# arunsethuraman/multiclust

Measured on AMD Instinct MI355X. Metric: EM iterations/sec, IxLxK admixture, higher is better.
Workload: dtype f64; 1 GPU; c3: 10000 diploid x 100000 loci, M_l~U{2,3,4}, admixture K=8, SQUAREM-3 (-s 3); I=10000, L=100000, T=300302, ploidy=2, K=8, accel_scheme=3, units=1 initialisation(s), one per GPU

## Files before the change

multiclust_amd/csrc/mchip.hip:

```cpp
#include "mchip_context.h"
#include "mchip_finalize.h"

#include <math.h>
#include <stdio.h>
#include <stdlib.h>
#include <string.h>
#include <sys/syscall.h>
#include <unistd.h>

mchip_progress_slot mchip_progress_slots[MCHIP_PROGRESS_SLOTS];
std::atomic<unsigned long long> mchip_progress_events{0};
static std::atomic<int> progress_next_slot{0};

mchip_progress_slot *mchip_progress_my_slot(void)
{
	static thread_local mchip_progress_slot *mine = nullptr;
	if (!mine) {
		int x = progress_next_slot.fetch_add(1, std::memory_order_relaxed);
		if (x >= MCHIP_PROGRESS_SLOTS) x = MCHIP_PROGRESS_SLOTS - 1;
		mine = &mchip_progress_slots[x];
		mine->tid.store((long)syscall(SYS_gettid), std::memory_order_relaxed);
	}
	return mine;
}
// ... 18 lines not shown
		mchip_ktable_get_17, mchip_ktable_get_18, mchip_ktable_get_19, mchip_ktable_get_20, mchip_ktable_get_21, mchip_ktable_get_22, mchip_ktable_get_23, mchip_ktable_get_24,
		mchip_ktable_get_25, mchip_ktable_get_26, mchip_ktable_get_27, mchip_ktable_get_28, mchip_ktable_get_29, mchip_ktable_get_30, mchip_ktable_get_31, mchip_ktable_get_32,
		mchip_ktable_get_33, mchip_ktable_get_34, mchip_ktable_get_35, mchip_ktable_get_36, mchip_ktable_get_37, mchip_ktable_get_38, mchip_ktable_get_39, mchip_ktable_get_40,
		mchip_ktable_get_41, mchip_ktable_get_42, mchip_ktable_get_43, mchip_ktable_get_44, mchip_ktable_get_45, mchip_ktable_get_46, mchip_ktable_get_47, mchip_ktable_get_48,
		mchip_ktable_get_49, mchip_ktable_get_50, mchip_ktable_get_51, mchip_ktable_get_52, mchip_ktable_get_53, mchip_ktable_get_54, mchip_ktable_get_55, mchip_ktable_get_56,
		mchip_ktable_get_57, mchip_ktable_get_58, mchip_ktable_get_59, mchip_ktable_get_60, mchip_ktable_get_61, mchip_ktable_get_62, mchip_ktable_get_63, mchip_ktable_get_64,
	};
	static_assert(MCHIP_MAX_K == 64, "one kernel translation unit per K (Makefile: KS)");
	return (K >= 1 && K <= MCHIP_MAX_K) ? tabs[K]() : nullptr;
}

static void read_knobs(mchip_context *ctx)
{
	auto on = [](const char *name) { return getenv(name) != nullptr ? 1 : 0; };
	auto num = [](const char *name, int dflt) { const char *e = getenv(name); return (e && atoi(e) > 0) ? atoi(e) : dflt; };
	ctx->knob.no_bial = on("MCHIP_NO_BIAL");
	ctx->knob.no_counts = on("MCHIP_NO_COUNTS");
	ctx->knob.force_dense = on("MCHIP_FORCE_DENSE");
	ctx->knob.force_safe = on("MCHIP_FORCE_SAFE");
	ctx->knob.no_graph = on("MCHIP_NO_GRAPH");
	ctx->knob.no_dual = on("MCHIP_NO_DUAL");
	ctx->knob.no_slab_sum = on("MCHIP_NO_SLAB_SUM");
	ctx->knob.no_fused_finalize = on("MCHIP_NO_FUSED_FINALIZE");
	ctx->knob.no_col_split = on("MCHIP_NO_COL_SPLIT");
	ctx->knob.part_no_tile = on("MCHIP_PART_NO_TILE");
	ctx->knob.sim_no_tile = on("MCHIP_SIM_NO_TILE");
	const int both = num("MCHIP_BLOCKS_PER_CU", 64);
	ctx->knob.per_cu_col = num("MCHIP_BLOCKS_PER_CU_COL", both);
	ctx->knob.per_cu_ind = num("MCHIP_BLOCKS_PER_CU_IND", both);
	const char *f = getenv("MCHIP_SLAB_FRAC");
	ctx->knob.slab_frac = (f && atof(f) > 0) ? atof(f) : 0.3;
	ctx->knob.no_roundup = on("MCHIP_NO_CHUNK_ROUNDUP");
	ctx->knob.geometry_given = on("MCHIP_BLOCKS_PER_CU") || on("MCHIP_BLOCKS_PER_CU_COL") || on("MCHIP_SLAB_FRAC");
}


constexpr int RT_I = 64;

__global__ __launch_bounds__(256) void k_relayout(const uint8_t *__restrict__ raw, int I, int L, int pl, const int32_t *__restrict__ ua,
			   int limit, uint8_t *gtA, uint8_t *gtS, int n_ltiles, int RT_L, int *bad)
{
	extern __shared__ __attribute__((aligned(16))) uint8_t tile[];
	const int rowb = RT_L * pl;
	const int l0 = (blockIdx.x % n_ltiles) * RT_L, i0 = (blockIdx.x / n_ltiles) * RT_I;
	int flags = 0;
	const int roww = rowb / 4;
// ... 747 lines not shown
	else { idx -= nq; pdst[idx] = cyc[1] ? p_if_accepted[idx] : p_otherwise[idx]; }
}

int check_slot(mchip_context *ctx, int slot)
{
	if (!ctx) return MCHIP_ERR_INVALID;
	if (!ctx->K) return fail(ctx, MCHIP_ERR_STATE, "no model set%s", nullptr);
	if (slot < 0 || slot > 2) return fail(ctx, MCHIP_ERR_INVALID, "slot out of range%s", nullptr);
	return MCHIP_OK;
}

static void prof_mark(mchip_context *ctx, int kind, bool start)
{
	if (!ctx->profiling) return;
	if (ctx->ev_used >= ctx->ev_pool.size()) {
		hipEvent_t e;
		if (hipEventCreate(&e) != hipSuccess) return;
		ctx->ev_pool.push_back(e);
	}
	(void)hipEventRecord(ctx->ev_pool[ctx->ev_used++], ctx->stream);
	if (start) ctx->ev_kind.push_back(kind);
}

static void drop_graphs(mchip_context *ctx)
{
	for (int s = 0; s < 3; s++)
		if (ctx->step_graph[s]) { (void)MCHIP_WAIT(hipGraphExecDestroy(ctx->step_graph[s])); ctx->step_graph[s] = nullptr; }
	for (int s = 0; s < 3; s++)
		for (int m = 0; m < 5; m++)
			if (ctx->cycle_graph[s][m]) { (void)MCHIP_WAIT(hipGraphExecDestroy(ctx->cycle_graph[s][m])); ctx->cycle_graph[s][m] = nullptr; }
}

void free_model(mchip_context *ctx)
{
	drop_graphs(ctx);
	for (int s = 0; s < 3; s++) { dfree(ctx->d_p[s]); dfree(ctx->d_q[s]); }
	for (int s = 0; s < MCHIP_MAX_SECANTS; s++) { dfree(ctx->d_up[s]); dfree(ctx->d_vp[s]); dfree(ctx->d_uq[s]); dfree(ctx->d_vq[s]); }
	dfree(ctx->d_sik); dfree(ctx->d_stage); dfree(ctx->d_logp); dfree(ctx->d_Apart); dfree(ctx->d_Spart); dfree(ctx->d_llpart); dfree(ctx->d_llpart2);
	dfree(ctx->d_redpart); dfree(ctx->d_flags);
	ctx->K = 0;
	ctx->parked_K = 0;
	ctx->kt = nullptr;
	ctx->have_ll = 0;
	ctx->s_cache_slot = -1;
}

// ... 98 lines not shown
	    MCHIP_WAIT(hipMalloc((void **)&ctx->d_run, sizeof(mchip_run_state))) != hipSuccess ||
	    MCHIP_WAIT(hipMalloc((void **)&ctx->d_cyc, 4 * sizeof(int))) != hipSuccess ||
	    MCHIP_WAIT(hipEventCreate(&ctx->ev_begin)) != hipSuccess || MCHIP_WAIT(hipEventCreate(&ctx->ev_end)) != hipSuccess) {
		delete ctx;
		return MCHIP_ERR_ALLOC;
	}
	*out = ctx;
	return MCHIP_OK;
}

int mchip_destroy(mchip_context *ctx)
{
	MCHIP_ENTRY();
	if (!ctx) return MCHIP_OK;
	(void)MCHIP_WAIT(hipSetDevice(ctx->device));
	(void)MCHIP_WAIT(hipStreamSynchronize(ctx->stream));
	free_model(ctx);
	free_data(ctx);
	dfree(ctx->d_scalars);
	dfree(ctx->d_cyc);
	dfree(ctx->d_run);
	if (ctx->h_pinned) (void)MCHIP_WAIT(hipHostFree(ctx->h_pinned));
	for (hipEvent_t e : ctx->ev_pool) (void)MCHIP_WAIT(hipEventDestroy(e));
	(void)MCHIP_WAIT(hipEventDestroy(ctx->ev_begin));
	(void)MCHIP_WAIT(hipEventDestroy(ctx->ev_end));
	(void)MCHIP_WAIT(hipStreamDestroy(ctx->stream));
	delete ctx;
	return MCHIP_OK;
}

const char *mchip_last_error(const mchip_context *ctx) { return ctx ? ctx->err : "null context"; }

int mchip_synchronize(mchip_context *ctx)
{
	MCHIP_ENTRY();
	if (!ctx) return MCHIP_ERR_INVALID;
	HIPCHK(hipStreamSynchronize(ctx->stream));
	return MCHIP_OK;
}

int mchip_device_info(mchip_context *ctx, char *name, int name_len, int *compute_units, double *hbm_bytes)
{
	MCHIP_ENTRY();
	if (!ctx) return MCHIP_ERR_INVALID;
	hipDeviceProp_t prop;
	HIPCHK(hipGetDeviceProperties(&prop, ctx->device));
// ... 597 lines not shown
		int rc = finalize_shared_eta(ctx, to, stop);
		if (rc) return rc;
		mchip_pass_args b = pass_args(ctx, from);
		b.Q = ctx->d_sik;
		b.qstride = ctx->K;
		b.stop = stop;
		prof_mark(ctx, MCHIP_KERN_ACCUM_P, true);
		ctx->kt->mix_column(b, ctx->stream);
		prof_mark(ctx, MCHIP_KERN_ACCUM_P, false);
		launch_finalize_p(ctx, ctx->kt->col_slabs(b, 1), ctx->d_Apart, from, to, 0, ctx->p_lb, ctx->do_projection, stop);
	}
	HIPCHK(hipGetLastError());
	if (mode == 0) ctx->have_ll = 1;
	return MCHIP_OK;
}

static int run_estep(mchip_context *ctx, int from, int to, int do_mstep, const int *stop = nullptr, const int *skip_ind = nullptr,
		     bool defer_ll = false)
{
	if (!ctx->admixture) return run_mixture(ctx, from, to, do_mstep, 0, stop, -1, defer_ll);
	mchip_pass_args a = pass_args(ctx, from);
	a.stop = stop;
	a.skip_ind = skip_ind;
	if (do_mstep || !ctx->sparse) {
		prof_mark(ctx, MCHIP_KERN_ACCUM_P, true);
		if (do_mstep) ctx->kt->accum_p(a, ctx->stream); else ctx->kt->loglik(a, ctx->stream);
		prof_mark(ctx, MCHIP_KERN_ACCUM_P, false);
	}
	if (ctx->sparse && do_mstep && !stop && ctx->s_cache_slot == from) {
		HIPCHK(hipMemcpyAsync(ctx->d_scalars, ctx->d_scalars + 2, sizeof(double), hipMemcpyDeviceToDevice, ctx->stream));
	} else {
		prof_mark(ctx, MCHIP_KERN_ACCUM_Q, true);
		ctx->kt->accum_q(a, ctx->stream);
		prof_mark(ctx, MCHIP_KERN_ACCUM_Q, false);
		ctx->ll_parts = ctx->kt->ind_ll_parts(a);
		if (!defer_ll)
			hipLaunchKernelGGL(k_reduce_sum, dim3(1), dim3(MCHIP_BLOCK), 0, ctx->stream, ctx->d_llpart, ctx->ll_parts, ctx->d_scalars, stop);
	}
	ctx->s_cache_slot = -1;
	const int indiv = ctx->qstride != 0;
	const int s_slabs = ctx->kt->ind_slabs(a), n_slabs = ctx->kt->col_slabs(a, 0);
	const int p_loci = finalize_p_loci(ctx->K, ctx->max_M);
	if (do_mstep && indiv && p_loci && !(n_slabs > 8 && !ctx->knob.no_slab_sum) && !ctx->knob.no_fused_finalize) {
		mchip_finalize_p_args p;
		p.L = ctx->L; p.K = ctx->K; p.T = ctx->T; p.loci_per_block = p_loci; p.n_slabs = n_slabs; p.weighted = 1;
		p.do_projection = ctx->do_projection; p.toff = ctx->d_toff; p.Apart = ctx->d_Apart; p.Pfrom = ctx->d_p[from];
		p.Pto = ctx->d_p[to]; p.add_lb = 0.0; p.lb = ctx->p_lb;
		ctx->kt->finalize_qp(ctx->I, s_slabs, ctx->d_Spart, ctx->d_q[from], ctx->qstride, ctx->d_q[to], ctx->d_sik,
				     ctx->do_projection, ctx->eta_lb, p, stop, ctx->stream);
		ctx->empty_rows_nan[to] = 1;
		HIPCHK(hipGetLastError());
		ctx->have_ll = 1;
// ... 587 lines not shown
	if (n_terms < 0 || (n_terms && (!v_index || !coef_a || !coef_b))) return MCHIP_ERR_INVALID;
	for (int t = 0; t < n_terms; t++) if ((rc = check_secant(ctx, v_index[t]))) return rc;
	HIPCHK(hipSetDevice(ctx->device));
	const size_t KT = (size_t)ctx->K * ctx->T;
	hipLaunchKernelGGL(k_add, dim3(nblk(KT)), dim3(256), 0, ctx->stream, ctx->d_p[base], ctx->d_up[u_index], ctx->d_p[to], KT);
	hipLaunchKernelGGL(k_add, dim3(nblk(ctx->nq)), dim3(256), 0, ctx->stream, ctx->d_q[base], ctx->d_uq[u_index], ctx->d_q[to], (size_t)ctx->nq);
	for (int t = 0; t < n_terms; t++) {
		hipLaunchKernelGGL(k_axpy2, dim3(nblk(KT)), dim3(256), 0, ctx->stream, ctx->d_vp[v_index[t]], ctx->d_p[to], KT, coef_a[t], coef_b[t]);
		hipLaunchKernelGGL(k_axpy2, dim3(nblk(ctx->nq)), dim3(256), 0, ctx->stream, ctx->d_vq[v_index[t]], ctx->d_q[to], (size_t)ctx->nq, coef_a[t], coef_b[t]);
	}
	HIPCHK(hipGetLastError());
	ctx->empty_rows_nan[to] = ctx->empty_rows_nan[base];
	return project_slot(ctx, to);
}

int mchip_profile_begin(mchip_context *ctx)
{
	MCHIP_ENTRY();
	if (!ctx) return MCHIP_ERR_INVALID;
	HIPCHK(hipSetDevice(ctx->device));
	ctx->profiling = 1;
	ctx->ev_used = 0;
	ctx->ev_kind.clear();
	HIPCHK(hipEventRecord(ctx->ev_begin, ctx->stream));
	return MCHIP_OK;
}

int mchip_profile_end(mchip_context *ctx, double *total_ms, double *kernel_ms, int *launches)
{
	MCHIP_ENTRY();
	if (!ctx) return MCHIP_ERR_INVALID;
	if (!ctx->profiling) return fail(ctx, MCHIP_ERR_STATE, "profile_end without profile_begin%s", nullptr);
	HIPCHK(hipSetDevice(ctx->device));
	HIPCHK(hipEventRecord(ctx->ev_end, ctx->stream));
	HIPCHK(hipEventSynchronize(ctx->ev_end));
	ctx->profiling = 0;
	float ms = 0;
	HIPCHK(hipEventElapsedTime(&ms, ctx->ev_begin, ctx->ev_end));
	if (total_ms) *total_ms = ms;
	double km[MCHIP_KERN_COUNT] = {0}, longest[MCHIP_KERN_COUNT] = {0};
	int kl[MCHIP_KERN_COUNT] = {0};
	std::vector<float> each(ctx->ev_kind.size(), 0.0f);
	for (size_t p = 0; 2 * p + 1 < ctx->ev_used && p < ctx->ev_kind.size(); p++) {
		HIPCHK(hipEventElapsedTime(&each[p], ctx->ev_pool[2 * p], ctx->ev_pool[2 * p + 1]));
		if (each[p] > longest[ctx->ev_kind[p]]) longest[ctx->ev_kind[p]] = each[p];
	}
	for (size_t p = 0; 2 * p + 1 < ctx->ev_used && p < ctx->ev_kind.size(); p++) {
		const int kind = ctx->ev_kind[p];
		if (each[p] < 0.05 * longest[kind]) continue;
		km[kind] += each[p];
		kl[kind]++;
	}
	for (int x = 0; x < MCHIP_KERN_COUNT; x++) {
		if (kernel_ms) kernel_ms[x] = km[x];
		if (launches) launches[x] = kl[x];
	}
	return MCHIP_OK;
}

int mchip_progress_note(const char *what)
{
	mchip_progress_slot *s = mchip_progress_my_slot();
	s->note.store(what, std::memory_order_relaxed);
	s->since_ns.store(mchip_progress_now(), std::memory_order_relaxed);
	mchip_progress_events.fetch_add(1, std::memory_order_relaxed);
	return MCHIP_OK;
}

int mchip_progress_report(char *buf, int buf_len, unsigned long long *events)
{
	if (events) *events = mchip_progress_events.load(std::memory_order_relaxed);
	if (!buf || buf_len <= 0) return MCHIP_OK;
// ... 20 lines not shown
```

multiclust_amd/csrc/mchip_context.h:

```cpp
#ifndef MCHIP_CONTEXT_H
#define MCHIP_CONTEXT_H

#include "mchip_internal.h"
#include "mchip_progress.h"

#include <functional>
#include <type_traits>
#include <stdio.h>
#include <string.h>

constexpr int RNG_LAG = 31;
constexpr int RNG_CHUNK = 4 * RNG_LAG * 32;

struct saved_set {
	uint8_t *d_raw = nullptr;
	int L = 0;
	std::vector<int32_t> ua;
	std::vector<int> empty;
};

struct mchip_context {
	int device;
	hipStream_t stream;
	char err[512];
// ... 29 lines not shown
	unsigned long long *d_cand_off;
	size_t cand_span_bytes, cand_loci, cand_center_bytes;
	uint32_t *d_jump_hi, *d_jump_lo;
	size_t n_jump_hi;
	struct lattice { uint32_t *d_i, *d_r; uint64_t A, B; unsigned nA, nB; } lat[2];
	uint32_t *d_part_slabs;
	size_t part_slab_bytes;
	uint8_t *d_sim_cluster;
	uint32_t *d_cen_part, *d_cen_work;
	size_t cen_part_bytes, cen_work_bytes;
	int K, admixture, constrained, do_projection, nsec, nq, qstride;
	double eta_lb, p_lb;
	const mchip_ktable *kt;
	double *d_p[3], *d_q[3];
	double *d_up[MCHIP_MAX_SECANTS], *d_vp[MCHIP_MAX_SECANTS], *d_uq[MCHIP_MAX_SECANTS], *d_vq[MCHIP_MAX_SECANTS];
	double *d_sik;
	double *d_stage;
	double *d_logp;
	int ichunk, n_ichunks, lchunk, n_lchunks, n_llpart, flush_blocks, safe_rcp, sparse;
	int ind_waves;
	int xcd_rows;
	struct {
		int no_bial, no_counts, force_dense, force_safe, no_graph, no_dual, no_slab_sum, no_col_split, part_no_tile, sim_no_tile;
		int no_fused_finalize;
		int per_cu_col, per_cu_ind, geometry_given, no_roundup;
		double slab_frac;
	} knob;
	double *d_Apart, *d_Spart, *d_llpart, *d_scalars;
	double *d_llpart2;
	double *d_redpart;
	uint8_t *d_flags;
	double *h_pinned;
	mchip_run_state *d_run;
	hipGraphExec_t step_graph[3];
	hipGraphExec_t cycle_graph[3][5];
	int *d_cyc;
	int have_ll;
	int ll_parts;
	int s_cache_slot;
	int profiling;
	hipEvent_t ev_begin, ev_end;
	std::vector<hipEvent_t> ev_pool;
	std::vector<int> ev_kind;
	size_t ev_used;
};

static int fail(mchip_context *ctx, int code, const char *fmt, const char *detail)
{
	if (ctx) snprintf(ctx->err, sizeof ctx->err, fmt, detail ? detail : "");
	return code;
}

#define HIPCHK(call)                                                                                  \
	do {                                                                                          \
		hipError_t e_ = MCHIP_WAIT(call);                                                     \
		if (e_ != hipSuccess) {                                                               \
			snprintf(ctx->err, sizeof ctx->err, "%s failed: %s (%s:%d)", #call,           \
				 hipGetErrorString(e_), __FILE__, __LINE__);                          \
			return MCHIP_ERR_HIP;                                                         \
		}                                                                                     \
	} while (0)

template <typename Tp> static void dfree(Tp *&p)
{
	if (p) (void)MCHIP_WAIT(hipFree(p));
	p = nullptr;
}
// ... 74 lines not shown
```

multiclust_amd/csrc/mchip_internal.h:

```cpp
#ifndef MCHIP_INTERNAL_H
#define MCHIP_INTERNAL_H

#include <hip/hip_runtime.h>
#include <stdint.h>
#include <vector>
#include "multiclust_hip.h"

#define MCHIP_BLOCK 256
#define MCHIP_SPARSE_MAX_M 32
#ifndef MCHIP_QBLOCK
#define MCHIP_QBLOCK 128
#endif

#ifdef MCHIP_FORCE_SPLIT1
constexpr int mchip_ind_split(int) { return 1; }
#else
constexpr int mchip_ind_split(int K) { return K <= 27 ? 1 : (K <= 48 ? 2 : 4); }
#endif
#ifdef MCHIP_FORCE_SPLIT1
constexpr int mchip_qblock(int) { return MCHIP_QBLOCK; }
#else
constexpr int mchip_qblock(int K) { return K > 48 ? 2 * MCHIP_QBLOCK : MCHIP_QBLOCK; }
#endif
#ifndef MCHIP_COL_SPLIT2_ABOVE
// ... 47 lines not shown
	const double *Q;
	int qstride;
	int ichunk, n_ichunks;
	double *Apart;
	double *llpart;
	int flush_blocks;
	int safe_rcp;
	int lchunk, n_lchunks;
	double *Spart;
	int xcd_rows;
	int no_col_split;
	int ind_waves;
	int sparse;
	int tile_cols;
	int biallelic;
	const int *stop;
	const int *skip_ind;
	const double *P2, *Q2;
	double *llpart2;
	const uint8_t *asA, *asS;
	int part_counts;
};

struct mchip_finalize_p_args {
	int L, K, T, loci_per_block, n_slabs, weighted, do_projection;
	const int32_t *toff;
	const double *Apart, *Pfrom;
	double *Pto;
	double add_lb, lb;
};

struct mchip_ktable {
	void (*accum_p)(const mchip_pass_args &a, hipStream_t s);
	void (*loglik)(const mchip_pass_args &a, hipStream_t s);
	void (*accum_q)(const mchip_pass_args &a, hipStream_t s);
	void (*part_p)(const mchip_pass_args &a, hipStream_t s);
	void (*part_q)(const mchip_pass_args &a, hipStream_t s);
	void (*finalize_q)(int I, int K, int n_lchunks, const double *Spart, const double *Qfrom, int qstride_from,
			   double *Qto, double *sik, int do_mstep, int weighted, int do_projection, double lb, const int *stop, hipStream_t s,
			   double add);
	void (*project_q)(int nrows, int K, double *Q, double lb, const int *stop, hipStream_t s);
	void (*mix_gather)(const mchip_pass_args &a, hipStream_t s);
	void (*mix_finalize)(int I, int n_lchunks, const double *Vpart, const double *eta, double *vik, double *llpart, int mode,
			     const int *stop, hipStream_t s);
	void (*mix_column)(const mchip_pass_args &a, hipStream_t s);
	int (*dual_available)(const mchip_pass_args &a);
	void (*accum_q_dual)(const mchip_pass_args &a, hipStream_t s);
	int (*col_slabs)(const mchip_pass_args &a, int mix);
	int (*ind_slabs)(const mchip_pass_args &a);
	int (*ind_ll_parts)(const mchip_pass_args &a);
	void (*finalize_qp)(int I, int n_slabs_q, const double *Spart, const double *Qfrom, int qstride_from, double *Qto, double *sik,
			    int do_projection_q, double lb_q, const mchip_finalize_p_args &p, const int *stop, hipStream_t s);
};

const mchip_ktable *mchip_get_ktable(int K);

inline int mchip_ind_waves(int K, int tile_cols)
{
	const size_t per_wave = (size_t)(K <= 12 ? 4 : 2) * ((((size_t)tile_cols * (size_t)mchip_kp(K) + 127) / 128) * 128) * sizeof(double);
	for (int w = MCHIP_IND_WAVES_MAX; w > 1; w >>= 1)
		if ((size_t)w * per_wave <= 48 * 1024) return w;
	return 1;
}
__host__ __device__ inline int mchip_ind_slabs(const mchip_pass_args &a) { return (a.n_lchunks + a.ind_waves - 1) / a.ind_waves; }
__host__ __device__ inline int mchip_col_slabs(const mchip_pass_args &a) { return (a.n_ichunks + MCHIP_COL_WAVES - 1) / MCHIP_COL_WAVES; }

#endif
```

multiclust_amd/csrc/mchip_kernels_k.hip:

```cpp
#include "mchip_internal.h"
#include "mchip_finalize.h"

#ifndef MCHIP_K
#error "compile with -DMCHIP_K=<K>"
#endif

namespace {

constexpr int K = MCHIP_K;

__device__ __forceinline__ double rcp_full(double t)
{
	const double r = __builtin_amdgcn_rcp(t);
	const double e = __builtin_fma(-t, r, 1.0);
	const double p = __builtin_fma(e, e, e);
	return __builtin_fma(r, p, r);
}

__device__ __forceinline__ void rcp4(const double (&t)[4], double (&rc)[4])
{
	const double p01 = t[0] * t[1], p23 = t[2] * t[3];
	const double rp = rcp_full(p01 * p23);
	const double r01 = rp * p23, r23 = rp * p01;
	rc[0] = r01 * t[1];
// ... 168 lines not shown
		if (LL && !SAFE) {
			if (++blk >= a.flush_blocks) {
				blk = 0;
				if (prod < 1e-100) {
					ll += log(prod);
					prod = 1.0;
				}
			}
		}
		g = gn;
	}
	if (ACCUM && valid) {
		double *out = a.Apart + ((size_t)blockIdx.y * a.T + c) * K;
#pragma unroll
		for (int k = 0; k < K; k++) out[k] = acc[k];
	}
	if (LL) {
		ll += log(prod);
		const double tot = block_sum<MCHIP_BLOCK>(ll, red);
		if (threadIdx.x == 0) a.llpart[(size_t)blockIdx.y * gridDim.x + blockIdx.x] = tot;
	}
}

template <int BITS, bool MIX, bool SAFE = false>
__global__ __launch_bounds__(MCHIP_BLOCK) void k_column_counts(mchip_pass_args a)
{
	if (a.stop && *a.stop) return;
	constexpr int PERWORD = 32 / BITS;
	constexpr int G = 4 * PERWORD;
	constexpr unsigned MASK = (1u << BITS) - 1u;
	constexpr int NJ = K <= 12 ? 4 : (K <= 20 ? 2 : 1);
	__shared__ double wsum[K][64];
	const int lane = threadIdx.x & 63, wv = threadIdx.x >> 6;
	const int c_raw = blockIdx.x * 64 + lane;
	const bool valid = c_raw < a.T;
	const int c = valid ? c_raw : a.T - 1;
	double p[K], acc[K];
#pragma unroll
	for (int k = 0; k < K; k++) {
		p[k] = MIX ? 0.0 : a.P[(size_t)c * K + k];
		acc[k] = 0.0;
	}
	const int i0 = __builtin_amdgcn_readfirstlane((blockIdx.y * MCHIP_COL_WAVES + wv) * a.ichunk);
	const int i1 = min(a.I, i0 + a.ichunk);
	const int g_end = (i1 + G - 1) / G;
	const uint4 *gt = reinterpret_cast<const uint4 *>(a.gtC);
	uint4 w = gt[(size_t)min(i0 / G, (a.I - 1) / G) * a.T + c];
	for (int g = i0 / G; g < g_end; g++) {
		const uint4 wn = gt[(size_t)min(g + 1, g_end - 1) * a.T + c];
#pragma unroll 1
		for (int wi = 0; wi < 4; wi++) {
			unsigned word = (wi == 0) ? w.x : (wi == 1) ? w.y : (wi == 2) ? w.z : w.w;
#pragma unroll 1
			for (int h = 0; h < PERWORD / NJ; h++) {
				const int ibase = g * G + wi * PERWORD + h * NJ;
				if (ibase >= i1) break;
				const double *__restrict__ q[NJ];
				double n[NJ], t[NJ], rc[NJ];
#pragma unroll
				for (int j = 0; j < NJ; j++) {
					q[j] = a.Q + (size_t)min(ibase + j, a.I - 1) * a.qstride;
					n[j] = (double)((word >> (BITS * j)) & MASK);
				}
				if (!MIX) {
#pragma unroll
					for (int j = 0; j < NJ; j++) {
						t[j] = q[j][0] * p[0];
#pragma unroll
						for (int k = 1; k < K; k++) t[j] = __builtin_fma(q[j][k], p[k], t[j]);
					}
					if (SAFE) {
#pragma unroll
						for (int j = 0; j < NJ; j++) rc[j] = (n[j] != 0.0) ? rcp_full(t[j]) : 0.0;
					} else {
						rcp_group(t, rc);
					}
				}
#pragma unroll
				for (int j = 0; j < NJ; j++) {
					const double r = MIX ? n[j] : n[j] * rc[j];
#pragma unroll
					for (int k = 0; k < K; k++) acc[k] = __builtin_fma(q[j][k], r, acc[k]);
				}
				word >>= NJ * BITS;
			}
		}
		w = wn;
	}
	unsigned tid = threadIdx.x;
	asm volatile("" : "+v"(tid));
	const int lane2 = (int)(tid & 63u), wv2 = (int)(tid >> 6);
	for (int x = 1; x < MCHIP_COL_WAVES; x++) {
		if (wv2 == x) {
#pragma unroll
			for (int k = 0; k < K; k++) wsum[k][lane2] = acc[k];
		}
		__syncthreads();
		if (wv2 == 0) {
#pragma unroll
			for (int k = 0; k < K; k++) acc[k] += wsum[k][lane2];
		}
		__syncthreads();
	}
	const int c2 = (int)blockIdx.x * 64 + lane2;
	if (wv2 == 0 && c2 < a.T) {
		double *out = a.Apart + ((size_t)blockIdx.y * a.T + c2) * K;
#pragma unroll
		for (int k = 0; k < K; k++) out[k] = acc[k];
	}
}

constexpr int CSPLIT = mchip_col_split(K);
constexpr int CKS = (K + CSPLIT - 1) / CSPLIT;
constexpr int CKSE = (CKS + 1) & ~1;
constexpr int cqs_stride(int n) { return ((2 * n) % 64 < 4 || (2 * n) % 64 > 60) ? n + 2 : n; }
constexpr int CQS = cqs_stride(CKSE + 2);

template <int CTRL> __device__ __forceinline__ double quad_exchange(double v)
{
	return __hiloint2double(__builtin_amdgcn_update_dpp(0, __double2hiint(v), CTRL, 0xF, 0xF, false),
				__builtin_amdgcn_update_dpp(0, __double2loint(v), CTRL, 0xF, 0xF, false));
}
__device__ __forceinline__ double quad_sum(double v)
{
	v += quad_exchange<0xB1>(v);
	if (CSPLIT == 4) v += quad_exchange<0x4E>(v);
	return v;
}

template <int BITS, bool SAFE>
__global__ __launch_bounds__(MCHIP_BLOCK) void k_column_counts_split(mchip_pass_args a)
{
// ... 448 lines not shown
#endif
__device__ __host__ __forceinline__ constexpr size_t tile_stride(int tile_cols)
{
	return GLDS ? (((size_t)tile_cols * KP + 127) / 128) * 128 : (size_t)tile_cols * KP;
}
typedef __attribute__((address_space(3))) double lds_double;
__device__ __forceinline__ void glds_copy(const double *src, lds_double *dst, int nel, int lane)
{
	const int units = nel >> 1;
	for (int u0 = 0; u0 < units; u0 += 64) {
		const double *g = src + 2 * (size_t)min(u0 + lane, units - 1);
		const unsigned l = __builtin_amdgcn_readfirstlane((unsigned)(size_t)(dst + 2 * (size_t)u0));
		unsigned keep;
		asm volatile("s_mov_b32 %0, m0\n\ts_mov_b32 m0, %2\n\ts_nop 0\n\tglobal_load_lds_dwordx4 %1, off\n\ts_mov_b32 m0, %0"
			     : "=&s"(keep) : "v"(g), "s"(l));
	}
}
__device__ __forceinline__ void glds_wait()
{
	asm volatile("s_waitcnt vmcnt(0)");
	__builtin_amdgcn_fence(__ATOMIC_ACQUIRE, "wavefront");
}

template <int PL, bool ACCUM, bool SAFE, bool NOMISS, bool DUAL = false>
__global__ __launch_bounds__(64 * MCHIP_IND_WAVES_MAX) void k_individual_sparse_w(mchip_pass_args a)
{
	static_assert(SPLIT == 1, "wave-private tiles: one lane per individual");
	static_assert(!DUAL || (ACCUM && !SAFE && PL == 2), "dual pass: ACCUM, shared reciprocals, diploid");
	if (a.stop && *a.stop) return;
	if (ACCUM && !DUAL && a.skip_ind && *a.skip_ind) return;
	extern __shared__ __attribute__((aligned(16))) double lds[];
	constexpr int SETS = DUAL ? 2 : 1;
	const int lane = threadIdx.x & 63;
	const int wv = __builtin_amdgcn_readfirstlane((int)(threadIdx.x >> 6));
	const int W = a.ind_waves;
	const int n_tiles = (a.I + 63) / 64;
	const int slot = a.xcd_rows ? (int)(blockIdx.x >> 3) : (int)blockIdx.x;
	const int bx = slot % n_tiles, by = a.xcd_rows ? (slot / n_tiles) * 8 + (int)(blockIdx.x & 7) : slot / n_tiles;
	const size_t tile_doubles = tile_stride(a.tile_cols);
	double *mine = lds + (size_t)wv * 2 * SETS * tile_doubles;
	const int i_raw = bx * 64 + lane;
	const bool active = i_raw < a.I;
	const int i = active ? i_raw : a.I - 1;
	const int pl = PL ? PL : a.ploidy;
	double q[K], acc[K], q2[DUAL ? K : 1];
#pragma unroll
	for (int k = 0; k < K; k++) {
		q[k] = a.Q[(size_t)i * a.qstride + k];
		acc[k] = 0.0;
		if constexpr (DUAL) q2[k] = a.Q2[(size_t)i * a.qstride + k];
	}
	const int l0 = (by * W + wv) * a.lchunk;
	const int l1 = min(a.L, l0 + a.lchunk);
	double prod = 1.0, prod2 = 1.0;
	int blk = 0, ex = 0, ex2 = 0;
	if (l0 < a.L) {
		if constexpr (!NOMISS) {
			for (size_t x = lane; x < 2 * SETS * tile_doubles; x += 64) mine[x] = 0.0;
		}
		const int lb0 = l0 >> 3, lb_end = (l1 + 7) >> 3;
		const bool staged = a.tile_cols * K <= WSTAGE * 64;
// ... 202 lines not shown
				if (DUAL) lds[(K + 1) * 64 + lane] = ll2;
			}
			__syncthreads();
			if (wv == 0) {
#pragma unroll
				for (int k = 0; k < K; k++) acc[k] += lds[k * 64 + lane];
				ll += lds[K * 64 + lane];
				if (DUAL) ll2 += lds[(K + 1) * 64 + lane];
			}
			__syncthreads();
		}
	}
	if (wv == 0) {
		if (ACCUM && active) {
			double *out = a.Spart + ((size_t)by * a.I + i) * K;
#pragma unroll
			for (int k = 0; k < K; k++) out[k] = acc[k];
		}
		const double tot = wave_total(active ? ll : 0.0);
		if (lane == 0) a.llpart[(size_t)by * n_tiles + bx] = tot;
		if (DUAL) {
			const double tot2 = wave_total(active ? ll2 : 0.0);
			if (lane == 0) a.llpart2[(size_t)by * n_tiles + bx] = tot2;
		}
	}
}

template <bool ACCUM, bool NOMISS>
__global__ __launch_bounds__(64 * MCHIP_IND_WAVES_MAX) void k_individual_bial(mchip_pass_args a)
{
	if (a.stop && *a.stop) return;
	if (ACCUM && a.skip_ind && *a.skip_ind) return;
	__shared__ double xch[K + 1][64];
	const int lane = threadIdx.x & 63;
	const int wv = __builtin_amdgcn_readfirstlane((int)(threadIdx.x >> 6));
	const int W = a.ind_waves;
	const int i_raw = blockIdx.x * 64 + lane;
	const bool active = i_raw < a.I;
	const int i = active ? i_raw : a.I - 1;
	double q[K], acc[K];
#pragma unroll
	for (int k = 0; k < K; k++) {
		q[k] = a.Q[(size_t)i * a.qstride + k];
		acc[k] = 0.0;
	}
	const int l0raw = (int)(blockIdx.y * W + wv) * a.lchunk;
// ... 530 lines not shown
			else if (!safe) hipLaunchKernelGGL((k_individual_sparse<PLV, ACCUM, false, false>), sparse_grid(a), dim3(QBLOCK), lds, s, a); \
			else hipLaunchKernelGGL((k_individual_sparse<PLV, ACCUM, true, false>), sparse_grid(a), dim3(QBLOCK), lds, s, a); \
		} while (0)
		if (a.ploidy == 2) MCHIP_SPARSE(2);
		else if (a.ploidy == 4) MCHIP_SPARSE(4);
		else hipLaunchKernelGGL((k_individual_sparse<0, ACCUM, true, false>), sparse_grid(a), dim3(QBLOCK), lds, s, a);
#undef MCHIP_SPARSE
	}
}
int dual_available(const mchip_pass_args &a)
{
	if (K > 12 || !a.sparse || a.flush_blocks < 1 || a.ploidy != 2) return 0;
	if (a.biallelic && K >= 6) return 0;
	return coop_lds_bytes(a, 2) <= 64 * 1024;
}
void launch_accum_q_dual(const mchip_pass_args &a, hipStream_t s)
{
	if constexpr (K <= 12) {
		const size_t lds = coop_lds_bytes(a, 2);
		if (!a.has_missing) hipLaunchKernelGGL((k_individual_sparse_w<2, true, false, true, true>), coop_rows(a), dim3(64 * a.ind_waves), lds, s, a);
		else hipLaunchKernelGGL((k_individual_sparse_w<2, true, false, false, true>), coop_rows(a), dim3(64 * a.ind_waves), lds, s, a);
	}
}
int col_slabs(const mchip_pass_args &a, int mix)
{
	if (mix) return a.count_bits ? mchip_col_slabs(a) : a.n_ichunks;
	return (a.sparse && a.count_bits && (CSPLIT == 1 || a.no_col_split)) ? mchip_col_slabs(a) : a.n_ichunks;
}
int ind_slabs(const mchip_pass_args &a) { return (a.sparse && SPLIT == 1) ? mchip_ind_slabs(a) : a.n_lchunks; }
int ind_ll_parts(const mchip_pass_args &a)
{
	if (a.sparse && SPLIT == 1) return ((a.I + 63) / 64) * mchip_ind_slabs(a);
	if (a.sparse) return ((a.I + QBLOCK / SPLIT - 1) / (QBLOCK / SPLIT)) * a.n_lchunks;
	return ((a.T + MCHIP_BLOCK - 1) / MCHIP_BLOCK) * a.n_ichunks;
}
void launch_loglik(const mchip_pass_args &a, hipStream_t s)
{
	if (a.sparse) { launch_sparse<false>(a, s); return; }
	if (a.ploidy == 2 && a.flush_blocks >= 1) hipLaunchKernelGGL((k_column_pass<2, false, false, true>), column_grid(a), dim3(MCHIP_BLOCK), 0, s, a);
	else if (a.ploidy == 2) hipLaunchKernelGGL((k_column_pass<2, false, true, true>), column_grid(a), dim3(MCHIP_BLOCK), 0, s, a);
	else hipLaunchKernelGGL((k_column_pass<0, false, true, true>), column_grid(a), dim3(MCHIP_BLOCK), 0, s, a);
}
void launch_accum_q(const mchip_pass_args &a, hipStream_t s)
{
	if (a.sparse) { launch_sparse<true>(a, s); return; }
	if (a.ploidy == 2) hipLaunchKernelGGL((k_individual_pass<2>), indiv_grid(a), dim3(QBLOCK), 0, s, a);
// ... 41 lines not shown
			   I, n_lchunks, Spart, Qfrom, qstride_from, Qto, sik, do_mstep, weighted, do_projection, lb, stop, add);
}
void launch_finalize_qp(int I, int n_lchunks, const double *Spart, const double *Qfrom, int qstride_from, double *Qto, double *sik,
			int do_projection_q, double lb_q, const mchip_finalize_p_args &p, const int *stop, hipStream_t s)
{
	const int q_blocks = (I + FQ_IND - 1) / FQ_IND, p_blocks = (p.L + p.loci_per_block - 1) / p.loci_per_block;
	hipLaunchKernelGGL(k_finalize_qp, dim3(q_blocks + p_blocks), dim3(MCHIP_BLOCK), 0, s,
			   q_blocks, I, n_lchunks, Spart, Qfrom, qstride_from, Qto, sik, do_projection_q, lb_q, p, stop);
}
void launch_project_q(int nrows, int, double *Q, double lb, const int *stop, hipStream_t s)
{
	hipLaunchKernelGGL(k_project_q, dim3((nrows + MCHIP_BLOCK - 1) / MCHIP_BLOCK), dim3(MCHIP_BLOCK), 0, s, nrows, Q, lb, stop);
}

}

#define MCHIP_CAT2(a, b) a##b
#define MCHIP_CAT(a, b) MCHIP_CAT2(a, b)
const mchip_ktable *MCHIP_CAT(mchip_ktable_get_, MCHIP_K)()
{
	static mchip_ktable t = {
		launch_accum_p, launch_loglik, launch_accum_q, launch_part_p, launch_part_q, launch_finalize_q, launch_project_q,
		launch_mix_gather, launch_mix_finalize, launch_mix_column, dual_available, launch_accum_q_dual,
		col_slabs, ind_slabs, ind_ll_parts, launch_finalize_qp,
	};
	return &t;
}
```

Measured before the change: 211.5 EM iterations/s.

## Fuse column-count and individual E-step passes into one interleaved paired launch

Adds a combined kernel that runs the column-count (P accumulation) and sparse individual (Q accumulation) bodies in one grid, interleaving runs of blocks of each kind so both passes share the device at once. This is meant to remove the serial dependency and tail idle time between the two separate launches and to let the two different resource profiles overlap. Q reads in the column body now go through the constant address space. The costs are a larger LDS allocation per block (the max of both bodies), possible register pressure from holding both code paths in one kernel, and extra per-block timing marks used only when profiling.

```diff
diff --git a/multiclust_amd/csrc/mchip.hip b/multiclust_amd/csrc/mchip.hip
--- a/multiclust_amd/csrc/mchip.hip
+++ b/multiclust_amd/csrc/mchip.hip
@@ -64,6 +64,7 @@
 	ctx->knob.no_dual = on("MCHIP_NO_DUAL");
 	ctx->knob.no_slab_sum = on("MCHIP_NO_SLAB_SUM");
 	ctx->knob.no_fused_finalize = on("MCHIP_NO_FUSED_FINALIZE");
+	ctx->knob.no_pair = on("MCHIP_NO_PAIR");
 	ctx->knob.no_col_split = on("MCHIP_NO_COL_SPLIT");
 	ctx->knob.part_no_tile = on("MCHIP_PART_NO_TILE");
 	ctx->knob.sim_no_tile = on("MCHIP_SIM_NO_TILE");
@@ -857,6 +858,63 @@
 	if (start) ctx->ev_kind.push_back(kind);
 }
 
+constexpr size_t PAIR_SPAN_CHUNK = 1024;
+constexpr int PAIR_SPAN_THREADS = 1024;
+__global__ __launch_bounds__(PAIR_SPAN_THREADS) void k_pair_spans(const unsigned long long *__restrict__ marks, unsigned n_blocks, mchip_pair_runs runs,
+								  mchip_pair_span *out)
+{
+	__shared__ unsigned long long red[4][PAIR_SPAN_THREADS];
+	unsigned long long lo[2] = { ~0ull, ~0ull }, hi[2] = { 0ull, 0ull };
+	for (unsigned r = threadIdx.x; r < n_blocks / MCHIP_PAIR_RUN; r += PAIR_SPAN_THREADS) {
+		unsigned logical;
+		const int kind = mchip_pair_is_ind(r * MCHIP_PAIR_RUN, runs, &logical) ? 1 : 0;
+#pragma unroll
+		for (int x = 0; x < MCHIP_PAIR_RUN; x++) {
+			const size_t b = (size_t)r * MCHIP_PAIR_RUN + x;
+			const unsigned long long t0 = marks[2 * b], t1 = marks[2 * b + 1];
+			if (t0 > t1) continue;
+			lo[kind] = t0 < lo[kind] ? t0 : lo[kind];
+			hi[kind] = t1 > hi[kind] ? t1 : hi[kind];
+		}
+	}
+	red[0][threadIdx.x] = lo[0]; red[1][threadIdx.x] = lo[1]; red[2][threadIdx.x] = hi[0]; red[3][threadIdx.x] = hi[1];
+	__syncthreads();
+	for (int s = PAIR_SPAN_THREADS / 2; s > 0; s >>= 1) {
+		if ((int)threadIdx.x < s) {
+			for (int x = 0; x < 2; x++) {
+				const unsigned long long l2 = red[x][threadIdx.x + s], h2 = red[2 + x][threadIdx.x + s];
+				if (l2 < red[x][threadIdx.x]) red[x][threadIdx.x] = l2;
+				if (h2 > red[2 + x][threadIdx.x]) red[2 + x][threadIdx.x] = h2;
+			}
+		}
+		__syncthreads();
+	}
+	if (threadIdx.x == 0) {
+		out->start[0] = red[0][0]; out->start[1] = red[1][0];
+		out->end[0] = red[2][0]; out->end[1] = red[3][0];
+	}
+}
+
+static int pair_profile_slot(mchip_context *ctx, const mchip_pass_args &a, unsigned long long **marks)
+{
+	mchip_pair_runs runs;
+	const size_t n_blocks = ctx->kt->pair_blocks(a, &runs);
+	if (n_blocks > ctx->pair_marks_cap) {
+		HIPCHK(hipStreamSynchronize(ctx->stream));
+		dfree(ctx->d_pair_marks);
+		ctx->pair_marks_cap = 0;
+		HIPCHK(hipMalloc((void **)&ctx->d_pair_marks, 2 * n_blocks * sizeof(unsigned long long)));
+		ctx->pair_marks_cap = n_blocks;
+	}
+	if (ctx->pair_used / PAIR_SPAN_CHUNK >= ctx->pair_spans.size()) {
+		mchip_pair_span *chunk = nullptr;
+		HIPCHK(hipMalloc((void **)&chunk, PAIR_SPAN_CHUNK * sizeof(mchip_pair_span)));
+		ctx->pair_spans.push_back(chunk);
+	}
+	*marks = ctx->d_pair_marks;
+	return MCHIP_OK;
+}
+
 static void drop_graphs(mchip_context *ctx)
 {
 	for (int s = 0; s < 3; s++)
@@ -1001,6 +1059,8 @@
 	dfree(ctx->d_run);
 	if (ctx->h_pinned) (void)MCHIP_WAIT(hipHostFree(ctx->h_pinned));
 	for (hipEvent_t e : ctx->ev_pool) (void)MCHIP_WAIT(hipEventDestroy(e));
+	dfree(ctx->d_pair_marks);
+	for (mchip_pair_span *&chunk : ctx->pair_spans) dfree(chunk);
 	(void)MCHIP_WAIT(hipEventDestroy(ctx->ev_begin));
 	(void)MCHIP_WAIT(hipEventDestroy(ctx->ev_end));
 	(void)MCHIP_WAIT(hipStreamDestroy(ctx->stream));
@@ -1644,12 +1704,33 @@
 	mchip_pass_args a = pass_args(ctx, from);
 	a.stop = stop;
 	a.skip_ind = skip_ind;
-	if (do_mstep || !ctx->sparse) {
+	const bool s_cached = ctx->sparse && do_mstep && !stop && ctx->s_cache_slot == from;
+	const bool paired = do_mstep && !s_cached && !ctx->knob.no_pair && ctx->kt->pair_available(a);
+	if (paired) {
+		unsigned long long *marks = nullptr;
+		if (ctx->profiling) {
+			int rc = pair_profile_slot(ctx, a, &marks);
+			if (rc) return rc;
+		}
+		ctx->kt->estep_pair(a, marks, ctx->stream);
+		if (marks) {
+			mchip_pair_runs runs;
+			const unsigned n_blocks = ctx->kt->pair_blocks(a, &runs);
+			hipLaunchKernelGGL(k_pair_spans, dim3(1), dim3(PAIR_SPAN_THREADS), 0, ctx->stream, marks, n_blocks, runs,
+					   ctx->pair_spans[ctx->pair_used / PAIR_SPAN_CHUNK] + ctx->pair_used % PAIR_SPAN_CHUNK);
+			ctx->pair_used++;
+		}
+		ctx->ll_parts = ctx->kt->ind_ll_parts(a);
+		if (!defer_ll)
+			hipLaunchKernelGGL(k_reduce_sum, dim3(1), dim3(MCHIP_BLOCK), 0, ctx->stream, ctx->d_llpart, ctx->ll_parts, ctx->d_scalars, stop);
+	}
+	if (!paired && (do_mstep || !ctx->sparse)) {
 		prof_mark(ctx, MCHIP_KERN_ACCUM_P, true);
 		if (do_mstep) ctx->kt->accum_p(a, ctx->stream); else ctx->kt->loglik(a, ctx->stream);
 		prof_mark(ctx, MCHIP_KERN_ACCUM_P, false);
 	}
-	if (ctx->sparse && do_mstep && !stop && ctx->s_cache_slot == from) {
+	if (paired) {
+	} else if (s_cached) {
 		HIPCHK(hipMemcpyAsync(ctx->d_scalars, ctx->d_scalars + 2, sizeof(double), hipMemcpyDeviceToDevice, ctx->stream));
 	} else {
 		prof_mark(ctx, MCHIP_KERN_ACCUM_Q, true);
@@ -2283,6 +2364,7 @@
 	ctx->profiling = 1;
 	ctx->ev_used = 0;
 	ctx->ev_kind.clear();
+	ctx->pair_used = 0;
 	HIPCHK(hipEventRecord(ctx->ev_begin, ctx->stream));
 	return MCHIP_OK;
 }
@@ -2302,13 +2384,29 @@
 	double km[MCHIP_KERN_COUNT] = {0}, longest[MCHIP_KERN_COUNT] = {0};
 	int kl[MCHIP_KERN_COUNT] = {0};
 	std::vector<float> each(ctx->ev_kind.size(), 0.0f);
-	for (size_t p = 0; 2 * p + 1 < ctx->ev_used && p < ctx->ev_kind.size(); p++) {
+	std::vector<int> kind_of(ctx->ev_kind);
+	for (size_t p = 0; 2 * p + 1 < ctx->ev_used && p < ctx->ev_kind.size(); p++)
 		HIPCHK(hipEventElapsedTime(&each[p], ctx->ev_pool[2 * p], ctx->ev_pool[2 * p + 1]));
-		if (each[p] > longest[ctx->ev_kind[p]]) longest[ctx->ev_kind[p]] = each[p];
-	}
-	for (size_t p = 0; 2 * p + 1 < ctx->ev_used && p < ctx->ev_kind.size(); p++) {
-		const int kind = ctx->ev_kind[p];
-		if (each[p] < 0.05 * longest[kind]) continue;
+	if (ctx->pair_used) {
+		int khz = 0;
+		if (MCHIP_WAIT(hipDeviceGetAttribute(&khz, hipDeviceAttributeWallClockRate, ctx->device)) != hipSuccess || khz <= 0) khz = 100000;
+		std::vector<mchip_pair_span> spans(ctx->pair_used);
+		for (size_t p = 0; p < ctx->pair_used; p += PAIR_SPAN_CHUNK) {
+			const size_t n = ctx->pair_used - p < PAIR_SPAN_CHUNK ? ctx->pair_used - p : PAIR_SPAN_CHUNK;
+			HIPCHK(hipMemcpy(&spans[p], ctx->pair_spans[p / PAIR_SPAN_CHUNK], n * sizeof(mchip_pair_span), hipMemcpyDeviceToHost));
+		}
+		for (const mchip_pair_span &sp : spans)
+			for (int x = 0; x < 2; x++) {
+				each.push_back(sp.end[x] > sp.start[x] ? (float)((double)(sp.end[x] - sp.start[x]) / khz) : 0.0f);
+				kind_of.push_back(x ? MCHIP_KERN_ACCUM_Q : MCHIP_KERN_ACCUM_P);
+			}
+		ctx->pair_used = 0;
+	}
+	for (size_t p = 0; p < each.size(); p++)
+		if (each[p] > longest[kind_of[p]]) longest[kind_of[p]] = each[p];
+	for (size_t p = 0; p < each.size(); p++) {
+		const int kind = kind_of[p];
+		if (each[p] <= 0.0f || each[p] < 0.05 * longest[kind]) continue;
 		km[kind] += each[p];
 		kl[kind]++;
 	}
diff --git a/multiclust_amd/csrc/mchip_context.h b/multiclust_amd/csrc/mchip_context.h
--- a/multiclust_amd/csrc/mchip_context.h
+++ b/multiclust_amd/csrc/mchip_context.h
@@ -75,7 +75,7 @@
 	int xcd_rows;
 	struct {
 		int no_bial, no_counts, force_dense, force_safe, no_graph, no_dual, no_slab_sum, no_col_split, part_no_tile, sim_no_tile;
-		int no_fused_finalize;
+		int no_fused_finalize, no_pair;
 		int per_cu_col, per_cu_ind, geometry_given, no_roundup;
 		double slab_frac;
 	} knob;
@@ -96,6 +96,10 @@
 	std::vector<hipEvent_t> ev_pool;
 	std::vector<int> ev_kind;
 	size_t ev_used;
+	unsigned long long *d_pair_marks;
+	size_t pair_marks_cap;
+	std::vector<mchip_pair_span *> pair_spans;
+	size_t pair_used;
 };
 
 static int fail(mchip_context *ctx, int code, const char *fmt, const char *detail)
diff --git a/multiclust_amd/csrc/mchip_internal.h b/multiclust_amd/csrc/mchip_internal.h
--- a/multiclust_amd/csrc/mchip_internal.h
+++ b/multiclust_amd/csrc/mchip_internal.h
@@ -93,6 +93,18 @@
 	int part_counts;
 };
 
+#define MCHIP_PAIR_RUN 8
+struct mchip_pair_runs { unsigned col_runs, ind_runs; };
+__host__ __device__ inline bool mchip_pair_is_ind(unsigned block, mchip_pair_runs r, unsigned *logical)
+{
+	const unsigned run = block / MCHIP_PAIR_RUN, total = r.col_runs + r.ind_runs;
+	const unsigned before = run * r.ind_runs / total, upto = (run + 1) * r.ind_runs / total;
+	const bool ind = upto > before;
+	*logical = (ind ? before : run - before) * MCHIP_PAIR_RUN + block % MCHIP_PAIR_RUN;
+	return ind;
+}
+struct mchip_pair_span { unsigned long long start[2], end[2]; };
+
 struct mchip_finalize_p_args {
 	int L, K, T, loci_per_block, n_slabs, weighted, do_projection;
 	const int32_t *toff;
@@ -122,6 +134,9 @@
 	int (*ind_ll_parts)(const mchip_pass_args &a);
 	void (*finalize_qp)(int I, int n_slabs_q, const double *Spart, const double *Qfrom, int qstride_from, double *Qto, double *sik,
 			    int do_projection_q, double lb_q, const mchip_finalize_p_args &p, const int *stop, hipStream_t s);
+	int (*pair_available)(const mchip_pass_args &a);
+	unsigned (*pair_blocks)(const mchip_pass_args &a, mchip_pair_runs *runs);
+	void (*estep_pair)(const mchip_pass_args &a, unsigned long long *marks, hipStream_t s);
 };
 
 const mchip_ktable *mchip_get_ktable(int K);
diff --git a/multiclust_amd/csrc/mchip_kernels_k.hip b/multiclust_amd/csrc/mchip_kernels_k.hip
--- a/multiclust_amd/csrc/mchip_kernels_k.hip
+++ b/multiclust_amd/csrc/mchip_kernels_k.hip
@@ -214,17 +214,15 @@
 	}
 }
 
-template <int BITS, bool MIX, bool SAFE = false>
-__global__ __launch_bounds__(MCHIP_BLOCK) void k_column_counts(mchip_pass_args a)
-{
-	if (a.stop && *a.stop) return;
+template <int BITS, bool MIX, bool SAFE>
+__device__ __forceinline__ void column_counts_body(const mchip_pass_args &a, const int bx, const int by, double (*wsum)[64])
+{
 	constexpr int PERWORD = 32 / BITS;
 	constexpr int G = 4 * PERWORD;
 	constexpr unsigned MASK = (1u << BITS) - 1u;
 	constexpr int NJ = K <= 12 ? 4 : (K <= 20 ? 2 : 1);
-	__shared__ double wsum[K][64];
 	const int lane = threadIdx.x & 63, wv = threadIdx.x >> 6;
-	const int c_raw = blockIdx.x * 64 + lane;
+	const int c_raw = bx * 64 + lane;
 	const bool valid = c_raw < a.T;
 	const int c = valid ? c_raw : a.T - 1;
 	double p[K], acc[K];
@@ -233,10 +231,12 @@
 		p[k] = MIX ? 0.0 : a.P[(size_t)c * K + k];
 		acc[k] = 0.0;
 	}
-	const int i0 = __builtin_amdgcn_readfirstlane((blockIdx.y * MCHIP_COL_WAVES + wv) * a.ichunk);
+	const int i0 = __builtin_amdgcn_readfirstlane((by * MCHIP_COL_WAVES + wv) * a.ichunk);
 	const int i1 = min(a.I, i0 + a.ichunk);
 	const int g_end = (i1 + G - 1) / G;
 	const uint4 *gt = reinterpret_cast<const uint4 *>(a.gtC);
+	typedef __attribute__((address_space(4))) double const_double;
+	const const_double *Qc = (const const_double *)a.Q;
 	uint4 w = gt[(size_t)min(i0 / G, (a.I - 1) / G) * a.T + c];
 	for (int g = i0 / G; g < g_end; g++) {
 		const uint4 wn = gt[(size_t)min(g + 1, g_end - 1) * a.T + c];
@@ -247,11 +247,11 @@
 			for (int h = 0; h < PERWORD / NJ; h++) {
 				const int ibase = g * G + wi * PERWORD + h * NJ;
 				if (ibase >= i1) break;
-				const double *__restrict__ q[NJ];
+				const const_double *q[NJ];
 				double n[NJ], t[NJ], rc[NJ];
 #pragma unroll
 				for (int j = 0; j < NJ; j++) {
-					q[j] = a.Q + (size_t)min(ibase + j, a.I - 1) * a.qstride;
+					q[j] = Qc + (size_t)min(ibase + j, a.I - 1) * a.qstride;
 					n[j] = (double)((word >> (BITS * j)) & MASK);
 				}
 				if (!MIX) {
@@ -294,12 +294,20 @@
 		}
 		__syncthreads();
 	}
-	const int c2 = (int)blockIdx.x * 64 + lane2;
+	const int c2 = bx * 64 + lane2;
 	if (wv2 == 0 && c2 < a.T) {
-		double *out = a.Apart + ((size_t)blockIdx.y * a.T + c2) * K;
+		double *out = a.Apart + ((size_t)by * a.T + c2) * K;
 #pragma unroll
 		for (int k = 0; k < K; k++) out[k] = acc[k];
 	}
+}
+
+template <int BITS, bool MIX, bool SAFE = false>
+__global__ __launch_bounds__(MCHIP_BLOCK) void k_column_counts(mchip_pass_args a)
+{
+	if (a.stop && *a.stop) return;
+	__shared__ double wsum[K][64];
+	column_counts_body<BITS, MIX, SAFE>(a, (int)blockIdx.x, (int)blockIdx.y, wsum);
 }
 
 constexpr int CSPLIT = mchip_col_split(K);
@@ -794,21 +802,18 @@
 	__builtin_amdgcn_fence(__ATOMIC_ACQUIRE, "wavefront");
 }
 
-template <int PL, bool ACCUM, bool SAFE, bool NOMISS, bool DUAL = false>
-__global__ __launch_bounds__(64 * MCHIP_IND_WAVES_MAX) void k_individual_sparse_w(mchip_pass_args a)
+template <int PL, bool ACCUM, bool SAFE, bool NOMISS, bool DUAL>
+__device__ __forceinline__ void individual_sparse_w_body(const mchip_pass_args &a, const unsigned bid, double *lds)
 {
 	static_assert(SPLIT == 1, "wave-private tiles: one lane per individual");
 	static_assert(!DUAL || (ACCUM && !SAFE && PL == 2), "dual pass: ACCUM, shared reciprocals, diploid");
-	if (a.stop && *a.stop) return;
-	if (ACCUM && !DUAL && a.skip_ind && *a.skip_ind) return;
-	extern __shared__ __attribute__((aligned(16))) double lds[];
 	constexpr int SETS = DUAL ? 2 : 1;
 	const int lane = threadIdx.x & 63;
 	const int wv = __builtin_amdgcn_readfirstlane((int)(threadIdx.x >> 6));
 	const int W = a.ind_waves;
 	const int n_tiles = (a.I + 63) / 64;
-	const int slot = a.xcd_rows ? (int)(blockIdx.x >> 3) : (int)blockIdx.x;
-	const int bx = slot % n_tiles, by = a.xcd_rows ? (slot / n_tiles) * 8 + (int)(blockIdx.x & 7) : slot / n_tiles;
+	const int slot = a.xcd_rows ? (int)(bid >> 3) : (int)bid;
+	const int bx = slot % n_tiles, by = a.xcd_rows ? (slot / n_tiles) * 8 + (int)(bid & 7) : slot / n_tiles;
 	const size_t tile_doubles = tile_stride(a.tile_cols);
 	double *mine = lds + (size_t)wv * 2 * SETS * tile_doubles;
 	const int i_raw = bx * 64 + lane;
@@ -1057,6 +1062,53 @@
 		if (DUAL) {
 			const double tot2 = wave_total(active ? ll2 : 0.0);
 			if (lane == 0) a.llpart2[(size_t)by * n_tiles + bx] = tot2;
+		}
+	}
+}
+
+template <int PL, bool ACCUM, bool SAFE, bool NOMISS, bool DUAL = false>
+__global__ __launch_bounds__(64 * MCHIP_IND_WAVES_MAX) void k_individual_sparse_w(mchip_pass_args a)
+{
+	if (a.stop && *a.stop) return;
+	if (ACCUM && !DUAL && a.skip_ind && *a.skip_ind) return;
+	extern __shared__ __attribute__((aligned(16))) double lds[];
+	individual_sparse_w_body<PL, ACCUM, SAFE, NOMISS, DUAL>(a, blockIdx.x, lds);
+}
+
+template <int BITS, int PL, bool SAFE, bool NOMISS>
+__global__ __launch_bounds__(MCHIP_BLOCK) void k_estep_pair(mchip_pass_args a, mchip_pair_runs runs, unsigned long long *marks)
+{
+	static_assert(64 * MCHIP_IND_WAVES_MAX == MCHIP_BLOCK, "both bodies at 256 threads");
+	extern __shared__ __attribute__((aligned(16))) double lds[];
+	unsigned logical;
+	const bool ind = mchip_pair_is_ind(blockIdx.x, runs, &logical);
+	const unsigned n_col = (unsigned)((a.T + 63) / 64), n_mine = ind ? (unsigned)(((a.I + 63) / 64) * mchip_ind_slabs(a)) : n_col * (unsigned)mchip_col_slabs(a);
+	const bool idle = logical >= n_mine || (a.stop && *a.stop) || (ind && a.skip_ind && *a.skip_ind);
+	if (idle) {
+		if (marks && threadIdx.x == 0) {
+			marks[2 * (size_t)blockIdx.x] = ~0ull;
+			marks[2 * (size_t)blockIdx.x + 1] = 0ull;
+		}
+		return;
+	}
+	const unsigned long long t_start = marks ? __builtin_amdgcn_s_memrealtime() : 0ull;
+	if (ind) individual_sparse_w_body<PL, true, SAFE, NOMISS, false>(a, logical, lds);
+	else column_counts_body<BITS, false, SAFE>(a, (int)(logical % n_col), (int)(logical / n_col), reinterpret_cast<double (*)[64]>(lds));
+	if (marks) {
+		unsigned long long (*wave_mark)[MCHIP_COL_WAVES] = reinterpret_cast<unsigned long long (*)[MCHIP_COL_WAVES]>(lds);
+		if ((threadIdx.x & 63) == 0) {
+			wave_mark[0][threadIdx.x >> 6] = t_start;
+			wave_mark[1][threadIdx.x >> 6] = __builtin_amdgcn_s_memrealtime();
+		}
+		__syncthreads();
+		if (threadIdx.x == 0) {
+			unsigned long long t0 = wave_mark[0][0], t1 = wave_mark[1][0];
+			for (int w = 1; w < MCHIP_COL_WAVES; w++) {
+				t0 = wave_mark[0][w] < t0 ? wave_mark[0][w] : t0;
+				t1 = wave_mark[1][w] > t1 ? wave_mark[1][w] : t1;
+			}
+			marks[2 * (size_t)blockIdx.x] = t0;
+			marks[2 * (size_t)blockIdx.x + 1] = t1;
 		}
 	}
 }
@@ -1633,6 +1685,37 @@
 		else hipLaunchKernelGGL((k_individual_sparse_w<2, true, false, false, true>), coop_rows(a), dim3(64 * a.ind_waves), lds, s, a);
 	}
 }
+unsigned pair_blocks(const mchip_pass_args &a, mchip_pair_runs *runs)
+{
+	const dim3 cg = counts_grid(a);
+	const unsigned n_col = cg.x * cg.y, n_ind = coop_rows(a).x;
+	runs->col_runs = (n_col + MCHIP_PAIR_RUN - 1) / MCHIP_PAIR_RUN;
+	runs->ind_runs = (n_ind + MCHIP_PAIR_RUN - 1) / MCHIP_PAIR_RUN;
+	return (runs->col_runs + runs->ind_runs) * MCHIP_PAIR_RUN;
+}
+int pair_available(const mchip_pass_args &a)
+{
+	if (K > 12 || SPLIT != 1 || CSPLIT != 1) return 0;
+	if (!a.sparse || a.count_bits != 2 || a.ploidy != 2 || a.ind_waves * 64 != MCHIP_BLOCK) return 0;
+	if ((a.safe_rcp != 0) != (a.flush_blocks < 1)) return 0;
+	if (a.biallelic && K >= 10 && a.flush_blocks >= 1) return 0;
+	mchip_pair_runs r;
+	pair_blocks(a, &r);
+	if (r.col_runs == 0 || r.ind_runs == 0) return 0;
+	return (unsigned long long)(r.col_runs + r.ind_runs) * r.ind_runs < (1ull << 32);
+}
+void launch_estep_pair(const mchip_pass_args &a, unsigned long long *marks, hipStream_t s)
+{
+	if constexpr (K <= 12 && SPLIT == 1 && CSPLIT == 1) {
+		mchip_pair_runs r;
+		const dim3 grid(pair_blocks(a, &r)), block(MCHIP_BLOCK);
+		const size_t ind_lds = coop_lds_bytes(a, 1), col_lds = (size_t)K * 64 * sizeof(double);
+		const size_t lds = ind_lds > col_lds ? ind_lds : col_lds;
+		if (a.flush_blocks < 1) hipLaunchKernelGGL((k_estep_pair<2, 2, true, false>), grid, block, lds, s, a, r, marks);
+		else if (!a.has_missing) hipLaunchKernelGGL((k_estep_pair<2, 2, false, true>), grid, block, lds, s, a, r, marks);
+		else hipLaunchKernelGGL((k_estep_pair<2, 2, false, false>), grid, block, lds, s, a, r, marks);
+	}
+}
 int col_slabs(const mchip_pass_args &a, int mix)
 {
 	if (mix) return a.count_bits ? mchip_col_slabs(a) : a.n_ichunks;
@@ -1720,7 +1803,7 @@
 	static mchip_ktable t = {
 		launch_accum_p, launch_loglik, launch_accum_q, launch_part_p, launch_part_q, launch_finalize_q, launch_project_q,
 		launch_mix_gather, launch_mix_finalize, launch_mix_column, dual_available, launch_accum_q_dual,
-		col_slabs, ind_slabs, ind_ll_parts, launch_finalize_qp,
+		col_slabs, ind_slabs, ind_ll_parts, launch_finalize_qp, pair_available, pair_blocks, launch_estep_pair,
 	};
 	return &t;
 }
```

New measurement: 220.2 EM iterations/s (median of 6 runs). 1.04x the previous value.
